# goalheart/ionic-mpnn

Hardware: AMD Instinct MI355X
Metric: molecule-graph pairs/sec (fwd), batch 4096 per MI355X (higher is better)
Workload: dtype f32 (bf16x9 emulation)

## Files before the change

### ionic_mpnn_amd/csrc/encoder_typed.hip

```cpp
#include "encoder_device.h"
#include "encoder_layout.h"

namespace impnn {
namespace enc {

namespace {

constexpr int kOffUpd = 0;
constexpr int off_h(bool x3) { return kOffUpd + (x3 ? kXUpdLds : kTUpdLds); }
constexpr int kTHSBig3 = 32;
constexpr int off_msg(bool x3, int hs = kTHS) { return off_h(x3) + kRCap * hs; }
constexpr int off_rec(bool x3, int ecap, int hs = kTHS) { return off_msg(x3, hs) + tmsg_floats(ecap); }
constexpr size_t lds_fixed_bytes(bool x3, int Vb, int ecap, int hs = kTHS) {
  return sizeof(float) * (size_t)off_rec(x3, ecap, hs) + trec_lds_bytes(Vb, ecap);
}
static_assert(lds_fixed_bytes(true, kTVbMax, kTECap) <= 160 * 1024 && lds_fixed_bytes(false, kTVbMax, kTECapBig) <= 160 * 1024 &&
                  lds_fixed_bytes(true, kTVbMax, kTECapBig, kTHSBig3) <= 160 * 1024,
              "LDS budget");

typedef __bf16 bf16x8 __attribute__((ext_vector_type(8)));
struct B3 {
  bf16x8 p0, p1, p2;
};
__device__ __forceinline__ void split_pair(float x, float y, unsigned& w0, unsigned& w1, unsigned& w2) {
  const unsigned xb = __builtin_bit_cast(unsigned, x), yb = __builtin_bit_cast(unsigned, y);
  const float x1 = x - __builtin_bit_cast(float, xb & 0xffff0000u), y1 = y - __builtin_bit_cast(float, yb & 0xffff0000u);
  const unsigned x1b = __builtin_bit_cast(unsigned, x1), y1b = __builtin_bit_cast(unsigned, y1);
  const float x2 = x1 - __builtin_bit_cast(float, x1b & 0xffff0000u), y2 = y1 - __builtin_bit_cast(float, y1b & 0xffff0000u);
  w0 = __builtin_amdgcn_perm(yb, xb, 0x07060302u);
  w1 = __builtin_amdgcn_perm(y1b, x1b, 0x07060302u);
  w2 = __builtin_amdgcn_perm(__builtin_bit_cast(unsigned, y2), __builtin_bit_cast(unsigned, x2), 0x07060302u);
}
__device__ __forceinline__ B3 split8x3(f32x4 a, f32x4 b) {
  union {
    bf16x8 v;
    unsigned u[4];
  } q0, q1, q2;
  split_pair(a[0], a[1], q0.u[0], q1.u[0], q2.u[0]);
  split_pair(a[2], a[3], q0.u[1], q1.u[1], q2.u[1]);
  split_pair(b[0], b[1], q0.u[2], q1.u[2], q2.u[2]);
  split_pair(b[2], b[3], q0.u[3], q1.u[3], q2.u[3]);
  B3 r;
  r.p0 = q0.v;
  r.p1 = q1.v;
  r.p2 = q2.v;
  return r;
}
__device__ __forceinline__ f32x4 mfmab(bf16x8 a, bf16x8 b, f32x4 c) {
  return __builtin_amdgcn_mfma_f32_16x16x32_bf16(a, b, c, 0, 0, 0);
}
__device__ __forceinline__ void mma9x2(f32x4& c0, f32x4& c1, const __bf16* blk0, const __bf16* blk1, int lane, const B3& b) {
  const bf16x8 a00 = *reinterpret_cast<const bf16x8*>(blk0 + lane * 8);
  const bf16x8 a01 = *reinterpret_cast<const bf16x8*>(blk0 + 512 + lane * 8);
  const bf16x8 a02 = *reinterpret_cast<const bf16x8*>(blk0 + 1024 + lane * 8);
  const bf16x8 a10 = *reinterpret_cast<const bf16x8*>(blk1 + lane * 8);
  const bf16x8 a11 = *reinterpret_cast<const bf16x8*>(blk1 + 512 + lane * 8);
  const bf16x8 a12 = *reinterpret_cast<const bf16x8*>(blk1 + 1024 + lane * 8);
  c0 = mfmab(a02, b.p2, c0);  c1 = mfmab(a12, b.p2, c1);
  c0 = mfmab(a01, b.p2, c0);  c1 = mfmab(a11, b.p2, c1);
  c0 = mfmab(a02, b.p1, c0);  c1 = mfmab(a12, b.p1, c1);
  c0 = mfmab(a00, b.p2, c0);  c1 = mfmab(a10, b.p2, c1);
  c0 = mfmab(a02, b.p0, c0);  c1 = mfmab(a12, b.p0, c1);
  c0 = mfmab(a01, b.p1, c0);  c1 = mfmab(a11, b.p1, c1);
  c0 = mfmab(a00, b.p1, c0);  c1 = mfmab(a10, b.p1, c1);
  c0 = mfmab(a01, b.p0, c0);  c1 = mfmab(a11, b.p0, c1);
  c0 = mfmab(a00, b.p0, c0);  c1 = mfmab(a10, b.p0, c1);
}

template <int ABID>
__device__ __forceinline__ f32x4 mfma1(float a, float b, f32x4 c) {
  return __builtin_amdgcn_mfma_f32_4x4x1f32(a, b, c, 3, ABID, 0);
}

typedef float f32x2v __attribute__((ext_vector_type(2)));
struct Grp {
  uint4 ge;
  f32x2v aq;
};
struct Run {
  f32x4 bq[4];
  Grp first;
};

__device__ __forceinline__ void group_messages(const f32x2v aq, const f32x4 (&bq)[4], float& m01, float& m23) {
  f32x4 acc0 = {0.f, 0.f, 0.f, 0.f}, acc1 = acc0;
#ifndef IMPNN_DIAG_NO_MSG_MFMA
  acc0 = mfma1<0>(aq[0], bq[0][0], acc0);
  acc1 = mfma1<0>(aq[1], bq[0][1], acc1);
  acc0 = mfma1<1>(aq[0], bq[0][2], acc0);
  acc1 = mfma1<1>(aq[1], bq[0][3], acc1);
  acc0 = mfma1<2>(aq[0], bq[1][0], acc0);
  acc1 = mfma1<2>(aq[1], bq[1][1], acc1);
  acc0 = mfma1<3>(aq[0], bq[1][2], acc0);
  acc1 = mfma1<3>(aq[1], bq[1][3], acc1);
  acc0 = mfma1<4>(aq[0], bq[2][0], acc0);
  acc1 = mfma1<4>(aq[1], bq[2][1], acc1);
  acc0 = mfma1<5>(aq[0], bq[2][2], acc0);
  acc1 = mfma1<5>(aq[1], bq[2][3], acc1);
  acc0 = mfma1<6>(aq[0], bq[3][0], acc0);
  acc1 = mfma1<6>(aq[1], bq[3][1], acc1);
  acc0 = mfma1<7>(aq[0], bq[3][2], acc0);
  acc1 = mfma1<7>(aq[1], bq[3][3], acc1);
#else
  acc0[0] = aq[0] + bq[0][0] + bq[3][3];
  acc1[1] = aq[1] + bq[1][1] + bq[2][2];
#endif
  float x0 = acc0[0] + acc1[0], x1 = acc0[1] + acc1[1], x2 = acc0[2] + acc1[2], x3 = acc0[3] + acc1[3];
  asm volatile("s_nop 1\n\tv_permlane32_swap_b32 %0, %1\n\tv_permlane32_swap_b32 %2, %3"
               : "+v"(x0), "+v"(x1), "+v"(x2), "+v"(x3));
  m01 = x0 + x1;
  m23 = x2 + x3;
}

__global__ __launch_bounds__(256) void typed_m0_kernel(const float* tmat0, const float* atom_table, float* m0,
                                                       M0Header* hdr, int Va, int Vb, int S) {
  const int lane = threadIdx.x & 63;
  const int w = __builtin_amdgcn_readfirstlane(blockIdx.x * 4 + (threadIdx.x >> 6));
  const int nga = (Va + 4) >> 2;
  if (w < Vb * nga) {
    const int v = w / nga, a0 = 4 * (w - v * nga);
    const int kh = lane >> 5, f = lane & 31;
    const int ai = a0 + (lane & 3);
    f32x2v aq = {0.f, 0.f};
    if (ai < Va) aq = *reinterpret_cast<const f32x2v*>(atom_table + (size_t)ai * kD + 16 * kh + 2 * ((lane >> 2) & 7));
    const float* bp = tmat0 + (size_t)v * kTMatFloats + kh * 512 + f * 4;
    f32x4 bq[4];
#pragma unroll
    for (int i = 0; i < 4; ++i) bq[i] = ld4(bp + i * 128);
    float m01, m23;
    group_messages(aq, bq, m01, m23);
    float* row = m0 + (size_t)v * (Va + 1) * kD + f;
    if (a0 + kh <= Va) row[(size_t)(a0 + kh) * kD] = m01;
    if (a0 + 2 + kh <= Va) row[(size_t)(a0 + 2 + kh) * kD] = m23;
  }
  if (blockIdx.x == 0 && threadIdx.x == 0) *hdr = M0Header{kM0Magic, Va, Vb, S};
}

#ifndef IMPNN_T_PF
#define IMPNN_T_PF 0
#endif
#ifndef IMPNN_T_EARLY
#define IMPNN_T_EARLY 0
#endif
constexpr int kPfWhere = IMPNN_T_PF, kRunsEarly = IMPNN_T_EARLY;

template <bool STAMPS, bool X3, int HS = kTHS>
__global__ __launch_bounds__(kThreads, kThreads / 256) void encoder_typed_kernel(TEncParams p) {
  extern __shared__ __align__(16) float smem[];
  constexpr int kUpdLds = X3 ? kXUpdLds : kTUpdLds, kUpdSlot = X3 ? kXUpdSlot : kTUpdSlot;
  constexpr int kNPf = X3 ? 3 : 2;
  float* const wupd = smem + kOffUpd;
  float* const wvec = wupd + (X3 ? kXVecFloatOff : kTVecFloatOff);
  float* const hbuf = smem + off_h(X3);
  float* const msg = smem + off_msg(X3, HS);
  const int zero_slot = p.ecap + 1;
  unsigned char* const recl = reinterpret_cast<unsigned char*>(smem + off_rec(X3, p.ecap, HS));
  const int rec_lds = p.rec_lds;
  float* const atab = reinterpret_cast<float*>(recl + rec_lds);
  const uint16_t* const r_rowdeg = reinterpret_cast<const uint16_t*>(recl + kTRecRowdeg);
  const unsigned char* const r_tilemax = recl + kTRecTilemax;
  const uint16_t* const r_moloff = reinterpret_cast<const uint16_t*>(recl + kTRecMoloff);
  const uint16_t* const r_molrows = reinterpret_cast<const uint16_t*>(recl + kTRecMolrows);
  const uint16_t* const r_poolrow = reinterpret_cast<const uint16_t*>(recl + kTRecPoolrow);
  const int32_t* const r_rowatom = reinterpret_cast<const int32_t*>(recl + kTRecRowatom);
  const uint16_t* const r_jdptr = reinterpret_cast<const uint16_t*>(recl + kTRecJdptr);
  const uint16_t* const r_runs = reinterpret_cast<const uint16_t*>(recl + trec_runs_off(p.Vb, p.ecap));
  int* const run_ctr = reinterpret_cast<int*>(recl + kTRecCounts + 8);
  const uint4* const r_grp = reinterpret_cast<const uint4*>(recl + kTRecGrp);

  const int tid = threadIdx.x, lane = tid & 63;
  const int wave = __builtin_amdgcn_readfirstlane(tid >> 6);
  const int a = lane & 15, q = lane >> 4;
  unsigned long long* stamp = STAMPS && p.stamps ? p.stamps + (size_t)blockIdx.x * 32 : nullptr;
  if (stamp && tid == 0) stamp[0] = __builtin_amdgcn_s_memtime();

  {
    const PlanHeader hd = *p.header;
    if (hd.magic != kPlanMagic || hd.kind != 1 || hd.nwg != (int)gridDim.x || hd.max_sub != p.max_sub ||
        hd.B != p.B || hd.n_ions != p.n_ions || hd.overflow != 0) {
      const float nan = __builtin_nanf("");
      for (int g = 0; g < p.n_ions; ++g)
        for (int64_t t = (int64_t)blockIdx.x * kThreads + tid; t < (int64_t)p.B * kD; t += (int64_t)gridDim.x * kThreads)
          p.pooled[g][t] = nan;
      return;
    }
  }
  const int c_begin = blockIdx.x * p.max_sub;
  const int c_end = c_begin + __builtin_amdgcn_readfirstlane(p.nsub[blockIdx.x]);
  if (c_begin >= c_end) return;

  if (p.atab_lds)
    for (int t = tid; t < (p.Va + 1) * (kTAS / 4); t += kThreads)
      st4(atab + 4 * t, t < p.Va * (kD / 4) ? ld4(p.atom_table + 4 * t) : f32x4{0.f, 0.f, 0.f, 0.f});
  if (tid < kD) msg[zero_slot * kD + tid] = 0.f;
  unsigned long long t_pro = 0, t_steps = 0, t_pool = 0, t_mark = 0, t_msg = 0;
  if (stamp && tid == 0) t_mark = __builtin_amdgcn_s_memtime();

  auto pool = [&](int M, int m0, int g) {
    float* out_g = p.pooled[g];
    for (int t0 = 0; t0 < M * 64; t0 += kThreads) {
      const int t = t0 + tid;
      const int part = t & 7, f4 = (t >> 3) & 7, m = t >> 6;
      f32x4 acc = {0.f, 0.f, 0.f, 0.f};
      if (m < M) {
        const int nr = r_molrows[m], mo = r_moloff[m];
        for (int n = part; n < nr; n += 8) {
          const int pr = r_poolrow[mo + n];
          if (pr & 0x8000) acc += ld4(hbuf + (pr & 0xff) * HS + 4 * f4);
        }
      }
#pragma unroll
      for (int i = 0; i < 4; ++i) {
        float v = acc[i];
        v += __builtin_bit_cast(float, __builtin_amdgcn_update_dpp(0, __builtin_bit_cast(int, v), 0xb1, 0xf, 0xf, true));
        v += __builtin_bit_cast(float, __builtin_amdgcn_update_dpp(0, __builtin_bit_cast(int, v), 0x4e, 0xf, 0xf, true));
        v += __builtin_bit_cast(float, __builtin_amdgcn_update_dpp(0, __builtin_bit_cast(int, v), 0x141, 0xf, 0xf, true));
        acc[i] = v;
      }
      if (m < M && part == 0) st4(out_g + (int64_t)(m0 + m) * kD + 4 * f4, acc);
    }
  };
  auto fill_h0 = [&]() {
    const int row = tid >> 2, sub = tid & 3;
    const int id = r_rowatom[row];
    f32x4 v0 = {0.f, 0.f, 0.f, 0.f}, v1 = v0;
    if ((unsigned)id < (unsigned)p.Va) {
      if (p.atab_lds) {
        v0 = ld4(atab + id * kTAS + 8 * sub);
        v1 = ld4(atab + id * kTAS + 8 * sub + 4);
      } else {
        v0 = ld4(p.atom_table + (int64_t)id * kD + 8 * sub);
        v1 = ld4(p.atom_table + (int64_t)id * kD + 8 * sub + 4);
      }
    }
    st4(hbuf + row * HS + 8 * sub, v0);
    st4(hbuf + row * HS + 8 * sub + 4, v1);
  };

  if (p.S == 0) {
    for (int c = c_begin; c < c_end; ++c) {
      const unsigned char* rc = p.rec + (size_t)c * kTRecBytes;
      if (8 * tid < rec_lds) reinterpret_cast<uint2*>(recl)[tid] = reinterpret_cast<const uint2*>(rc)[tid];
      const int4 dsc = reinterpret_cast<const int4*>(p.desc)[c];
      lds_barrier();
      fill_h0();
      lds_barrier();
      pool(__builtin_amdgcn_readfirstlane(dsc.y), __builtin_amdgcn_readfirstlane(dsc.x),
           __builtin_amdgcn_readfirstlane(dsc.w) >> 16);
      lds_barrier();
    }
    return;
  }

  unsigned tabmask = 0;
  {
    const M0Header t0 = *reinterpret_cast<const M0Header*>(p.upd[0] + kUpdLds);
    if (t0.magic == kM0Magic && t0.Va == p.Va && t0.Vb == p.Vb && t0.S == p.S) tabmask |= 1u;
    if (p.n_ions > 1) {
      const M0Header t1 = *reinterpret_cast<const M0Header*>(p.upd[1] + kUpdLds);
      if (t1.magic == kM0Magic && t1.Va == p.Va && t1.Vb == p.Vb && t1.S == p.S) tabmask |= 2u;
    }
  }

  const bool rec_big = rec_lds > kTRecPart1;
  const unsigned char* rec_c = p.rec + (size_t)c_begin * kTRecBytes;
  uint2 rec_n8 = reinterpret_cast<const uint2*>(rec_c)[tid];
  uint32_t rec_n4 = rec_big ? reinterpret_cast<const uint32_t*>(rec_c + kTRecPart1)[tid] : 0u;
  int4 dsc_next = reinterpret_cast<const int4*>(p.desc)[c_begin];

  const uint32_t* const grp_x = reinterpret_cast<const uint32_t*>(r_grp);
  const int kh = lane >> 5, f = lane & 31;
  const int boff = kh * 512 + f * 4;
  const int ysh = 8 * (lane & 3), zsh = 16 * kh;
  const int acol = 16 * kh + 2 * ((lane >> 2) & 7);

  for (int c = c_begin; c < c_end; ++c) {
    const int4 dsc = dsc_next;
    const int m0 = __builtin_amdgcn_readfirstlane(dsc.x), M = __builtin_amdgcn_readfirstlane(dsc.y);
    const int rg = __builtin_amdgcn_readfirstlane(dsc.w);
    const int R = rg & 0xffff, g = rg >> 16;
    const int ntiles = (R + 15) >> 4;
    const float* upd_g = p.upd[g];
    const float* tmat_g = p.tmat[g];
    const bool tab0 = (tabmask >> g) & 1u;
    if (8 * tid < rec_lds) reinterpret_cast<uint2*>(recl)[tid] = rec_n8;
    if (rec_big && kTRecPart1 + 4 * tid < rec_lds) reinterpret_cast<uint32_t*>(recl + kTRecPart1)[tid] = rec_n4;
    {
      const int cn = (c + 1) < c_end ? (c + 1) : c;
      const unsigned char* rn = p.rec + (size_t)cn * kTRecBytes;
      rec_n8 = reinterpret_cast<const uint2*>(rn)[tid];
      if (rec_big) rec_n4 = reinterpret_cast<const uint32_t*>(rn + kTRecPart1)[tid];
      dsc_next = reinterpret_cast<const int4*>(p.desc)[cn];
    }
    lds_barrier();
    fill_h0();
    if (tab0) {
      const int ngrp = __builtin_amdgcn_readfirstlane(*reinterpret_cast<const uint16_t*>(recl + kTRecCounts));
      const float* const m0_g = p.m0[g];
      int tl = tid;
      asm volatile("" : "+v"(tl));
      const unsigned u4 = 4 * (tl & 7);
      const int i = (tl >> 3) & 3, g0 = tl >> 5;
      constexpr int kGR = 8;
      const unsigned dump = (unsigned)tmsg_key(p.ecap);
      for (int gb = 0; gb < ngrp; gb += 32 * kGR) {
        f32x4 mv[kGR];
        unsigned dst[kGR];
#pragma unroll
        for (int j = 0; j < kGR; ++j) {
          const int gi = gb + 32 * j + g0;
          const uint4 ge = r_grp[gi < ngrp ? gi : ngrp - 1];
          const bool ok = gi < ngrp && i < (int)__builtin_amdgcn_ubfe(ge.x, 8, 8);
          const int id = r_rowatom[__builtin_amdgcn_ubfe(ge.y, 8 * i, 8)];
          const unsigned col = (unsigned)id < (unsigned)p.Va ? (unsigned)id : (unsigned)p.Va;
          const unsigned off = ((ge.x & 0xffu) * (unsigned)(p.Va + 1) + col) * kD + u4;
          mv[j] = ld4(m0_g + (ok ? off : 0u));
          dst[j] = (ok ? __builtin_amdgcn_ubfe(i < 2 ? ge.z : ge.w, 16 * (i & 1), 16) : dump) ^ u4;
        }
#pragma unroll
        for (int j = 0; j < kGR; ++j) st4(msg + dst[j], mv[j]);
      }
    }
    if (tid == 0) *run_ctr = 2 * kWaves;
    lds_barrier();
    if (stamp && tid == 0) {
      const unsigned long long t = __builtin_amdgcn_s_memtime();
      t_pro += t - t_mark;
      t_mark = t;
    }
    const int nrun = __builtin_amdgcn_readfirstlane(*reinterpret_cast<const uint16_t*>(recl + kTRecNrun));

    Run P, Q;
    int gP = 0, nP = 0, gQ = 0, nQ = 0;
    bool haveP = false, haveQ = false;
    const bool sP = wave < nrun, sQ = wave + kWaves < nrun;
    const int sgP = __builtin_amdgcn_readfirstlane(r_runs[sP ? wave : 0]);
    const int snP = __builtin_amdgcn_readfirstlane(r_runs[(sP ? wave : 0) + 1]) - sgP;
    const int sgQ = __builtin_amdgcn_readfirstlane(r_runs[sQ ? wave + kWaves : 0]);
    const int snQ = __builtin_amdgcn_readfirstlane(r_runs[(sQ ? wave + kWaves : 0) + 1]) - sgQ;
    const int soP = sP ? (__builtin_amdgcn_readfirstlane(grp_x[4 * sgP]) & 0xff) * kTMatFloats : 0;
    const int soQ = sQ ? (__builtin_amdgcn_readfirstlane(grp_x[4 * sgQ]) & 0xff) * kTMatFloats : 0;
    const int lboffP = sP ? boff : 0, lboffQ = sQ ? boff : 0;
    f32x4 pf[kNPf];
    auto fetch_pf = [&](int s_) {
#pragma unroll
      for (int i = 0; i < kNPf; ++i) pf[i] = ld4(upd_g + (int64_t)s_ * kUpdSlot + 4 * (tid + i * kThreads));
    };
    auto fetch_P = [&](int s_) {
      const float* tm = tmat_g + (size_t)s_ * p.Vb * kTMatFloats;
#pragma unroll
      for (int i = 0; i < 4; ++i) P.bq[i] = ld4(tm + soP + lboffP + i * 128);
    };
    auto fetch_Q = [&](int s_) {
      const float* tm = tmat_g + (size_t)s_ * p.Vb * kTMatFloats;
#pragma unroll
      for (int i = 0; i < 4; ++i) Q.bq[i] = ld4(tm + soQ + lboffQ + i * 128);
    };
    if (kPfWhere != 0) fetch_pf(0);
    if (kRunsEarly >= 1) fetch_P(0);
    if (kRunsEarly >= 2) fetch_Q(0);
    if (stamp && c == c_begin && tid == 0) stamp[13] = __builtin_amdgcn_s_memtime();
    for (int s = 0; s < p.S; ++s) {
      const float* tm_s = tmat_g + (size_t)s * p.Vb * kTMatFloats;
      __builtin_amdgcn_s_setprio(2);
      const bool from_tab = tab0 && s == 0;
      if (kPfWhere == 0) fetch_pf(s);
      if (!from_tab) {
        const float* const abase = hbuf + acol;
        auto load_group = [&](int e, Grp& G) {
          G.ge = r_grp[e];
          const int src = __builtin_amdgcn_ubfe(G.ge.y, ysh, 8);
          G.aq = *reinterpret_cast<const f32x2v*>(abase + src * HS);
        };
        auto compute = [&](const Grp& G, const f32x4 (&bq)[4]) {
          float m01, m23;
          group_messages(G.aq, bq, m01, m23);
          msg[__builtin_amdgcn_ubfe(G.ge.z, zsh, 16) ^ f] = m01;
          msg[__builtin_amdgcn_ubfe(G.ge.w, zsh, 16) ^ f] = m23;
        };
        auto run_type = [&](int g_, int n_, Run& Rn) {
          const int end = g_ + n_;
          Grp T;
          int e = g_;
          while (true) {
            if (e + 1 < end) load_group(e + 1, T);
            compute(Rn.first, Rn.bq);
            if (++e >= end) break;
            if (e + 1 < end) load_group(e + 1, Rn.first);
            compute(T, Rn.bq);
            if (++e >= end) break;
          }
        };
        auto fetch = [&](bool have, int r, int& g_, int& n_, Run& Rn, const float* tm) {
          const int rc = have ? r : 0;
          g_ = __builtin_amdgcn_readfirstlane(r_runs[rc]);
          n_ = __builtin_amdgcn_readfirstlane(r_runs[rc + 1]) - g_;
          const int type = have ? (__builtin_amdgcn_readfirstlane(grp_x[4 * g_]) & 0xff) : 0;
          const float* bp = tm + (size_t)type * kTMatFloats + (have ? boff : 0);
#pragma unroll
          for (int i = 0; i < 4; ++i) Rn.bq[i] = ld4(bp + i * 128);
        };
        auto next_run = [&]() {
          int r = 0;
          if (lane == 0) r = atomicAdd(run_ctr, 1);
          return __builtin_amdgcn_readfirstlane(r);
        };
        auto take = [&](int r, int& g_, int& n_, Run& Rn) {
          fetch(true, r, g_, n_, Rn, tm_s);
          load_group(g_, Rn.first);
        };
        auto landed = [](f32x4 (&b)[4]) {
          asm volatile("" : "+v"(b[0]), "+v"(b[1]), "+v"(b[2]), "+v"(b[3]) : : "memory");
        };
        if (kRunsEarly < 1) fetch_P(s);
        if (kRunsEarly < 2) fetch_Q(s);
        haveP = sP; gP = sgP; nP = snP;
        haveQ = sQ; gQ = sgQ; nQ = snQ;
        if (haveP) load_group(gP, P.first);
        if (haveQ) load_group(gQ, Q.first);
        if (haveP) {
          if (!haveQ) {
            landed(P.bq);
            run_type(gP, nP, P);
          } else {
            while (true) {
              landed(P.bq);
              run_type(gP, nP, P);
              const int rP = next_run();
              if (rP >= nrun) {
                landed(Q.bq);
                run_type(gQ, nQ, Q);
                break;
              }
              take(rP, gP, nP, P);
              landed(Q.bq);
              run_type(gQ, nQ, Q);
              const int rQ = next_run();
              if (rQ >= nrun) {
                landed(P.bq);
                run_type(gP, nP, P);
                break;
              }
              take(rQ, gQ, nQ, Q);
            }
          }
        }
      }
#pragma unroll
      for (int i = 0; i < kNPf; ++i)
        if (4 * (tid + i * kThreads) < kUpdLds) st4(wupd + 4 * (tid + i * kThreads), pf[i]);
      const bool mstamp = stamp && c == c_begin && s == 1;
      if (mstamp && lane == 0) stamp[16 + wave] = __builtin_amdgcn_s_memtime();
      lds_barrier();
      if (tid == 0) *run_ctr = 2 * kWaves;
      if (mstamp && tid == 0) stamp[12] = __builtin_amdgcn_s_memtime();
      if (stamp && tid == 0 && c == c_begin && s == 1) t_msg = __builtin_amdgcn_s_memtime();

      int my_tile = -1;
      {
        const int grp = wave & 3, slot = wave >> 2, q4 = ntiles >> 2, r4 = ntiles & 3;
        const int heavy = (4 - r4) * q4;
        if (grp >= r4) {
          if (slot < q4) my_tile = slot * (4 - r4) + (grp - r4);
        } else if (slot <= q4) {
          my_tile = heavy + slot * r4 + grp;
        }
      }
      const bool has_tile = my_tile >= 0 && my_tile < ntiles;
      if (has_tile) {
        const int tile = my_tile;
        const int row = tile * 16 + a;
        const int deg = r_rowdeg[row];
        const int maxdeg = __builtin_amdgcn_readfirstlane(r_tilemax[tile]);
        f32x4 agg0 = {0.f, 0.f, 0.f, 0.f}, agg1 = agg0;
        for (int d0 = 0; d0 < maxdeg; d0 += 4) {
          const uint2 jd = *reinterpret_cast<const uint2*>(r_jdptr + d0);
          int sl[4];
          sl[0] = d0 + 0 < deg ? (int)(jd.x & 0xffffu) + row : zero_slot;
          sl[1] = d0 + 1 < deg ? (int)(jd.x >> 16) + row : zero_slot;
          sl[2] = d0 + 2 < deg ? (int)(jd.y & 0xffffu) + row : zero_slot;
          sl[3] = d0 + 3 < deg ? (int)(jd.y >> 16) + row : zero_slot;
          f32x4 m0v[4], m1v[4];
#pragma unroll
          for (int j = 0; j < 4; ++j) {
            const int o = tmsg_off(sl[j], q);
            m0v[j] = ld4(msg + o);
            m1v[j] = ld4(msg + (o ^ 16));
          }
#pragma unroll
          for (int j = 0; j < 4; ++j) {
            agg0 += m0v[j];
            agg1 += m1v[j];
          }
        }
        if (mstamp && wave == 1 && lane == 0) stamp[8] = __builtin_amdgcn_s_memtime();
        __builtin_amdgcn_s_setprio(1);
        if (s + 1 < p.S) {
          if (kPfWhere == 1) fetch_pf(s + 1);
          if (kRunsEarly >= 1) fetch_P(s + 1);
          if (kRunsEarly >= 2) fetch_Q(s + 1);
        }
        const f32x4 h0 = ld4(hbuf + row * HS + 4 * q);
        const f32x4 h1 = ld4(hbuf + row * HS + 16 + 4 * q);

        f32x4 z0 = ld4(wvec + 0 * kD + 4 * q), z1 = ld4(wvec + 0 * kD + 16 + 4 * q);
        f32x4 r0 = ld4(wvec + 1 * kD + 4 * q), r1 = ld4(wvec + 1 * kD + 16 + 4 * q);
        f32x4 t0 = ld4(wvec + 2 * kD + 4 * q), t1 = ld4(wvec + 2 * kD + 16 + 4 * q);
        if constexpr (X3) {
          const __bf16* wb = reinterpret_cast<const __bf16*>(wupd);
          const B3 sh = split8x3(h0, h1);
          const B3 sa = split8x3(agg0, agg1);
          mma9x2(z0, z1, wb + ((0 * 2 + 0) * 2 + 0) * 1536, wb + ((0 * 2 + 1) * 2 + 0) * 1536, lane, sh);
          mma9x2(r0, r1, wb + ((1 * 2 + 0) * 2 + 0) * 1536, wb + ((1 * 2 + 1) * 2 + 0) * 1536, lane, sh);
          mma9x2(z0, z1, wb + ((0 * 2 + 0) * 2 + 1) * 1536, wb + ((0 * 2 + 1) * 2 + 1) * 1536, lane, sa);
          mma9x2(r0, r1, wb + ((1 * 2 + 0) * 2 + 1) * 1536, wb + ((1 * 2 + 1) * 2 + 1) * 1536, lane, sa);
          z0 = sigmoid4<false>(z0);
          z1 = sigmoid4<false>(z1);
          const f32x4 rh0 = sigmoid4<false>(r0) * h0;
          const f32x4 rh1 = sigmoid4<false>(r1) * h1;
          const B3 srh = split8x3(rh0, rh1);
          mma9x2(t0, t1, wb + ((2 * 2 + 0) * 2 + 0) * 1536, wb + ((2 * 2 + 1) * 2 + 0) * 1536, lane, srh);
          mma9x2(t0, t1, wb + ((2 * 2 + 0) * 2 + 1) * 1536, wb + ((2 * 2 + 1) * 2 + 1) * 1536, lane, sa);
        } else {
          const float* wl = wupd + 4 * lane;
#pragma unroll
          for (int half = 0; half < 2; ++half) {
#pragma unroll
            for (int u = 0; u < 2; ++u) {
              const int hu = half * 2 + u;
              const f32x4 Az0 = ld4(wl + ((0 * 2 + 0) * 4 + hu) * 256);
              const f32x4 Az1 = ld4(wl + ((0 * 2 + 1) * 4 + hu) * 256);
              const f32x4 Ar0 = ld4(wl + ((1 * 2 + 0) * 4 + hu) * 256);
              const f32x4 Ar1 = ld4(wl + ((1 * 2 + 1) * 4 + hu) * 256);
              const f32x4 Bv = half == 0 ? (u == 0 ? h0 : h1) : (u == 0 ? agg0 : agg1);
#pragma unroll
              for (int r = 0; r < 4; ++r) {
                z0 = mfma4(Az0[r], Bv[r], z0);
                z1 = mfma4(Az1[r], Bv[r], z1);
                r0 = mfma4(Ar0[r], Bv[r], r0);
                r1 = mfma4(Ar1[r], Bv[r], r1);
              }
            }
          }
          z0 = sigmoid4<false>(z0);
          z1 = sigmoid4<false>(z1);
          const f32x4 rh0 = sigmoid4<false>(r0) * h0;
          const f32x4 rh1 = sigmoid4<false>(r1) * h1;
#pragma unroll
          for (int half = 0; half < 2; ++half) {
#pragma unroll
            for (int u = 0; u < 2; ++u) {
              const int hu = half * 2 + u;
              const f32x4 Ah0 = ld4(wl + ((2 * 2 + 0) * 4 + hu) * 256);
              const f32x4 Ah1 = ld4(wl + ((2 * 2 + 1) * 4 + hu) * 256);
              const f32x4 Bv = half == 0 ? (u == 0 ? rh0 : rh1) : (u == 0 ? agg0 : agg1);
#pragma unroll
              for (int r = 0; r < 4; ++r) {
                t0 = mfma4(Ah0[r], Bv[r], t0);
                t1 = mfma4(Ah1[r], Bv[r], t1);
              }
            }
          }
        }
        __builtin_amdgcn_s_setprio(0);
        if (kPfWhere == 2 && s + 1 < p.S) {
          asm volatile("" ::: "memory");
          fetch_pf(s + 1);
        }
        if (mstamp && wave == 1 && lane == 0) stamp[9] = __builtin_amdgcn_s_memtime();
        f32x4 n0 = z0 * (tanh4<false>(t0) - h0) + h0;
        f32x4 n1 = z1 * (tanh4<false>(t1) - h1) + h1;
        const f32x4 s4 = n0 + n1;
        float sum = (s4[0] + s4[1]) + (s4[2] + s4[3]);
        sum += __shfl_xor(sum, 16);
        sum += __shfl_xor(sum, 32);
        const float mean = sum * (1.0f / kD);
        n0 -= mean;
        n1 -= mean;
        const f32x4 q4 = n0 * n0 + n1 * n1;
        float var = (q4[0] + q4[1]) + (q4[2] + q4[3]);
        var += __shfl_xor(var, 16);
        var += __shfl_xor(var, 32);
        const float inv = __builtin_amdgcn_rsqf(var * (1.0f / kD) + p.ln_eps);
        const f32x4 gm0 = ld4(wvec + 3 * kD + 4 * q), gm1 = ld4(wvec + 3 * kD + 16 + 4 * q);
        const f32x4 bt0 = ld4(wvec + 4 * kD + 4 * q), bt1 = ld4(wvec + 4 * kD + 16 + 4 * q);
        const f32x4 o0 = n0 * (gm0 * inv) + (bt0 + h0);
        const f32x4 o1 = n1 * (gm1 * inv) + (bt1 + h1);
        st4(hbuf + row * HS + 4 * q, o0);
        st4(hbuf + row * HS + 16 + 4 * q, o1);
        if (mstamp && wave == 1 && lane == 0) stamp[10] = __builtin_amdgcn_s_memtime();
      }
      if (!has_tile && s + 1 < p.S) {
        if (kPfWhere != 0) fetch_pf(s + 1);
        if (kRunsEarly >= 1) fetch_P(s + 1);
        if (kRunsEarly >= 2) fetch_Q(s + 1);
      }
      if (mstamp && wave == 1 && lane == 0) stamp[11] = __builtin_amdgcn_s_memtime();
      lds_barrier();
      if (stamp && c == c_begin && s < 2 && tid == 0) stamp[14 + s] = __builtin_amdgcn_s_memtime();
    }
    if (stamp && tid == 0) {
      const unsigned long long t = __builtin_amdgcn_s_memtime();
      t_steps += t - t_mark;
      t_mark = t;
    }

    pool(M, m0, g);
    lds_barrier();
    if (stamp && tid == 0) {
      const unsigned long long t = __builtin_amdgcn_s_memtime();
      t_pool += t - t_mark;
      t_mark = t;
    }
  }
  if (stamp && tid == 0) {
    stamp[1] = t_pro;
    stamp[2] = t_steps;
    stamp[3] = t_pool;
    stamp[4] = (unsigned long long)(c_end - c_begin);
    stamp[5] = t_msg;
    stamp[7] = __builtin_amdgcn_s_memtime();
  }
}

}
}

bool encoder_typed_supported(int N, int E, int D, int S, int Vb) {
  using namespace enc;
  if (D != kD || S < 0) return false;
  if (N < 1 || N > 0xffff || E < 0 || E > 0xffff) return false;
  if (Vb < 1 || Vb > kTVbMax) return false;
  return true;
}

size_t encoder_typed_prepared_bytes(int S, int Vb, bool x3) {
  return enc::typed_prepared_floats(S, Vb, x3) * sizeof(float);
}

int launch_encoder_typed_prepare(const float* weights, const float* bond_table, int K, int S, int Vb, bool x3,
                                 void* prepared, hipStream_t s) {
  if (S <= 0) return IMPNN_OK;
  enc::TImageParams ip{};
  ip.weights = weights;
  ip.bond_table = bond_table;
  ip.prepared = static_cast<float*>(prepared);
  ip.K = K;
  ip.S = S;
  ip.Vb = Vb;
  ip.x3 = x3 ? 1 : 0;
  ip.step_floats = impnn_encoder_step_floats(enc::kD, K);
  return enc::launch_typed_image(ip, s);
}

size_t encoder_typed_prepared_bytes_atoms(int S, int Va, int Vb, bool x3) {
  return (enc::typed_prepared_floats(S, Vb, x3) + enc::m0_table_floats(S, Va, Vb)) * sizeof(float);
}

int launch_encoder_typed_prepare_atoms(const float* weights, const float* bond_table, const float* atom_table, int Va,
                                       int K, int S, int Vb, bool x3, void* prepared, hipStream_t s) {
  using namespace enc;
  if (int rc = launch_encoder_typed_prepare(weights, bond_table, K, S, Vb, x3, prepared, s)) return rc;
  if (m0_table_floats(S, Va, Vb) == 0) return IMPNN_OK;
  float* img = static_cast<float*>(prepared);
  const size_t uslot = x3 ? kXUpdSlot : kTUpdSlot;
  const int waves = Vb * ((Va + 4) >> 2);
  typed_m0_kernel<<<(waves + 3) / 4, 256, 0, s>>>(img + (size_t)S * uslot, atom_table, img + typed_prepared_floats(S, Vb, x3),
                                                  reinterpret_cast<M0Header*>(img + (x3 ? kXUpdLds : kTUpdLds)), Va, Vb, S);
  return check_launch("typed_m0");
}

int launch_encoder_typed_run(const EncoderArgs& a, const enc::Ws& w, hipStream_t s) {
  using namespace enc;
  char* base = static_cast<char*>(a.workspace);
  TEncParams ep{};
  const size_t S1 = a.S > 0 ? a.S : 1;
  const bool x3 = a.mode == 3;
  const size_t uslot = x3 ? kXUpdSlot : kTUpdSlot;
  for (int g = 0; g < a.n_ions; ++g) {
    const float* prep;
    if (a.prepared[g]) {
      if (!aligned16(a.prepared[g])) return fail(IMPNN_E_BADARG, "encoder_fused: prepared weights must be 16B aligned");
      prep = static_cast<const float*>(a.prepared[g]);
    } else {
      float* img = reinterpret_cast<float*>(base + w.img_off) + (size_t)g * typed_prepared_floats(a.S, a.Vb, x3);
      if (int rc = launch_encoder_typed_prepare(a.weights[g], a.bond_table, a.K, a.S, a.Vb, x3, img, s)) return rc;
      prep = img;
    }
    ep.upd[g] = prep;
    ep.tmat[g] = prep + S1 * uslot;
    ep.m0[g] = prep + typed_prepared_floats(a.S, a.Vb, x3);
    ep.pooled[g] = a.pooled[g];
  }
  ep.atom_table = a.atom_table;
  ep.nsub = reinterpret_cast<const int32_t*>(base + w.nsub_off);
  ep.desc = reinterpret_cast<const int32_t*>(base + w.desc_off);
  ep.rec = reinterpret_cast<const unsigned char*>(base + w.rec_off);
  ep.header = reinterpret_cast<const PlanHeader*>(base);
  ep.n_ions = a.n_ions; ep.B = a.B; ep.S = a.S; ep.Va = a.Va; ep.Vb = a.Vb; ep.max_sub = w.max_sub;
  ep.ln_eps = a.ln_eps;
  ep.stamps = nullptr;
  {
    size_t sb = 0;
    void* sp = debug_stamp_buffer(&sb);
    if (sp && sb >= (size_t)w.nwg * 32 * sizeof(unsigned long long)) ep.stamps = static_cast<unsigned long long*>(sp);
  }
  ep.upd_slot = (int)uslot;
  ep.ecap = tecap_of(a.E);
  ep.rec_lds = trec_lds_bytes(a.Vb, ep.ecap);
  const bool big3 = x3 && ep.ecap == kTECapBig;
  void (*kern)(TEncParams) =
      big3 ? (ep.stamps ? encoder_typed_kernel<true, true, kTHSBig3> : encoder_typed_kernel<false, true, kTHSBig3>)
      : x3 ? (ep.stamps ? encoder_typed_kernel<true, true> : encoder_typed_kernel<false, true>)
           : (ep.stamps ? encoder_typed_kernel<true, false> : encoder_typed_kernel<false, false>);
  if (int rc = ensure_lds_limit((const void*)kern, big3 ? (ep.stamps ? 10 : 9) : (ep.stamps ? 5 : 4) + (x3 ? 2 : 0))) return rc;
  size_t lds = lds_fixed_bytes(x3, a.Vb, ep.ecap, big3 ? kTHSBig3 : kTHS);
  const size_t atab_bytes = ((size_t)a.Va + 1) * kTAS * sizeof(float);
  ep.atab_lds = lds + atab_bytes <= 160 * 1024;
  if (ep.atab_lds) lds += atab_bytes;
  profile_record_start(s);
  kern<<<w.nwg, kThreads, lds, s>>>(ep);
  profile_record_stop(s);
  return check_launch("encoder_typed");
}

}
```

Measured before the change: 37.58 million.

## DMA step-0 update weights into LDS with global_load_lds, overlapping prologue and pooling

Loads the step-0 update weight image straight from global memory into LDS with global_load_lds_dwordx4. The load is issued during the prologue for the first subgraph and before pooling for each following one, so the register prefetch and LDS store at s==0 are skipped. The barrier before the update phase is dropped when step 0 uses the precomputed table. This hides the weight transfer behind other work, but relies on inline asm that touches m0 and on explicit vmcnt waits, which may be fragile around LDS hazards.

```diff
diff --git a/ionic_mpnn_amd/csrc/encoder_typed.hip b/ionic_mpnn_amd/csrc/encoder_typed.hip
--- a/ionic_mpnn_amd/csrc/encoder_typed.hip
+++ b/ionic_mpnn_amd/csrc/encoder_typed.hip
@@ -136,6 +136,16 @@
   if (blockIdx.x == 0 && threadIdx.x == 0) *hdr = M0Header{kM0Magic, Va, Vb, S};
 }
 
+__device__ __forceinline__ void glds16(const float* gsrc, const float* lds_dst) {
+  const unsigned dst = __builtin_amdgcn_readfirstlane(
+      (unsigned)(uintptr_t)(__attribute__((address_space(3))) const void*)lds_dst);
+  unsigned keep;
+  asm volatile("s_mov_b32 %0, m0\n\ts_mov_b32 m0, %2\n\ts_nop 0\n\tglobal_load_lds_dwordx4 %1, off\n\ts_mov_b32 m0, %0"
+               : "=&s"(keep)
+               : "v"(gsrc), "s"(dst)
+               : "memory");
+}
+
 #ifndef IMPNN_T_PF
 #define IMPNN_T_PF 0
 #endif
@@ -149,6 +159,7 @@
   extern __shared__ __align__(16) float smem[];
   constexpr int kUpdLds = X3 ? kXUpdLds : kTUpdLds, kUpdSlot = X3 ? kXUpdSlot : kTUpdSlot;
   constexpr int kNPf = X3 ? 3 : 2;
+  static_assert(kXUpdLds % 256 == 0 && kTUpdLds % 256 == 0, "the update image is copied in 1 KiB pieces (dma_upd0)");
   float* const wupd = smem + kOffUpd;
   float* const wvec = wupd + (X3 ? kXVecFloatOff : kTVecFloatOff);
   float* const hbuf = smem + off_h(X3);
@@ -189,6 +200,15 @@
   const int c_end = c_begin + __builtin_amdgcn_readfirstlane(p.nsub[blockIdx.x]);
   if (c_begin >= c_end) return;
 
+  auto retire_vm = []() { __builtin_amdgcn_s_waitcnt(0x0f70); };
+  auto dma_upd0 = [&](int g_) {
+    const float* src = p.upd[g_] + 4 * lane;
+#pragma unroll
+    for (int i = 0; i < kNPf; ++i) {
+      const int pc = wave + kWaves * i;
+      if (pc * 256 < kUpdLds) glds16(src + pc * 256, wupd + pc * 256);
+    }
+  };
   if (p.atab_lds)
     for (int t = tid; t < (p.Va + 1) * (kTAS / 4); t += kThreads)
       st4(atab + 4 * t, t < p.Va * (kD / 4) ? ld4(p.atom_table + 4 * t) : f32x4{0.f, 0.f, 0.f, 0.f});
@@ -221,7 +241,9 @@
     }
   };
   auto fill_h0 = [&]() {
-    const int row = tid >> 2, sub = tid & 3;
+    int tl = tid;
+    asm volatile("" : "+v"(tl));
+    const int row = tl >> 2, sub = tl & 3;
     const int id = r_rowatom[row];
     f32x4 v0 = {0.f, 0.f, 0.f, 0.f}, v1 = v0;
     if ((unsigned)id < (unsigned)p.Va) {
@@ -267,6 +289,8 @@
   uint2 rec_n8 = reinterpret_cast<const uint2*>(rec_c)[tid];
   uint32_t rec_n4 = rec_big ? reinterpret_cast<const uint32_t*>(rec_c + kTRecPart1)[tid] : 0u;
   int4 dsc_next = reinterpret_cast<const int4*>(p.desc)[c_begin];
+  retire_vm();
+  dma_upd0(__builtin_amdgcn_readfirstlane(dsc_next.w) >> 16);
 
   const uint32_t* const grp_x = reinterpret_cast<const uint32_t*>(r_grp);
   const int kh = lane >> 5, f = lane & 31;
@@ -322,6 +346,7 @@
       }
     }
     if (tid == 0) *run_ctr = 2 * kWaves;
+    asm volatile("s_waitcnt vmcnt(0)" ::: "memory");
     lds_barrier();
     if (stamp && tid == 0) {
       const unsigned long long t = __builtin_amdgcn_s_memtime();
@@ -356,7 +381,6 @@
 #pragma unroll
       for (int i = 0; i < 4; ++i) Q.bq[i] = ld4(tm + soQ + lboffQ + i * 128);
     };
-    if (kPfWhere != 0) fetch_pf(0);
     if (kRunsEarly >= 1) fetch_P(0);
     if (kRunsEarly >= 2) fetch_Q(0);
     if (stamp && c == c_begin && tid == 0) stamp[13] = __builtin_amdgcn_s_memtime();
@@ -364,7 +388,14 @@
       const float* tm_s = tmat_g + (size_t)s * p.Vb * kTMatFloats;
       __builtin_amdgcn_s_setprio(2);
       const bool from_tab = tab0 && s == 0;
-      if (kPfWhere == 0) fetch_pf(s);
+      if (kPfWhere == 0) {
+        if (s > 0) {
+          fetch_pf(s);
+        } else {
+#pragma unroll
+          for (int i = 0; i < kNPf; ++i) pf[i] = f32x4{0.f, 0.f, 0.f, 0.f};
+        }
+      }
       if (!from_tab) {
         const float* const abase = hbuf + acol;
         auto load_group = [&](int e, Grp& G) {
@@ -446,12 +477,14 @@
           }
         }
       }
-#pragma unroll
-      for (int i = 0; i < kNPf; ++i)
-        if (4 * (tid + i * kThreads) < kUpdLds) st4(wupd + 4 * (tid + i * kThreads), pf[i]);
+      if (s > 0) {
+#pragma unroll
+        for (int i = 0; i < kNPf; ++i)
+          if (4 * (tid + i * kThreads) < kUpdLds) st4(wupd + 4 * (tid + i * kThreads), pf[i]);
+      }
       const bool mstamp = stamp && c == c_begin && s == 1;
       if (mstamp && lane == 0) stamp[16 + wave] = __builtin_amdgcn_s_memtime();
-      lds_barrier();
+      if (!from_tab) lds_barrier();
       if (tid == 0) *run_ctr = 2 * kWaves;
       if (mstamp && tid == 0) stamp[12] = __builtin_amdgcn_s_memtime();
       if (stamp && tid == 0 && c == c_begin && s == 1) t_msg = __builtin_amdgcn_s_memtime();
@@ -605,6 +638,8 @@
       t_mark = t;
     }
 
+    retire_vm();
+    if (c + 1 < c_end) dma_upd0(__builtin_amdgcn_readfirstlane(dsc_next.w) >> 16);
     pool(M, m0, g);
     lds_barrier();
     if (stamp && tid == 0) {
```

Measured after the change: 37.49 million. About the same (-0.2%).
